# debbiemarkslab/BEAR

Measured on AMD Instinct MI355X. Metric: k-mer contexts/sec (DM-marginal+grad h), k=13, higher is better.
Workload: dtype f64

## Files before the change

### bear_amd/csrc/bear_hip.hip

```cpp
#include "bear_host.h"
#include "kernels_finalize.h"
#include "kernels_rows.h"
#include "kernels_sorted.h"
#include "kernels_plan.h"
#include "kernels_synth.h"
#include "kernels_refmix.h"
#include "kernels_mixplan.h"
#include "kernels_sample.h"
#include "kernels_shuffle.h"
#include "kernels_refplan.h"

#ifdef PLN_STAMPS
#define PLN_DBG_ARG , ws->dbg
#else
#define PLN_DBG_ARG
#endif

extern "C" {

int bear_abi_version(void) { return BEAR_ABI_VERSION; }

const char *bear_strerror(int status) {
  switch (status) {
    case BEAR_OK: return "ok";
// ... 361 lines not shown

static int plan_count_live_rows(bear_plan *p, const plan_scan &sc) {
  unsigned long long h_hist[SRT_NKEY];
  HIP_TRY(hipMemcpy(h_hist, p->hist, sizeof(h_hist), hipMemcpyDeviceToHost));
  unsigned long long live_rows = sc.heavy[1];
  for (int k = 0; k < SRT_NKEY; ++k) live_rows += h_hist[k];
  p->n_live_rows = live_rows;
  return BEAR_OK;
}

static int plan_build(const bear_ws *ws, bear_plan *p) {
  plan_scan sc;
  plan_cut cut;
  int st = plan_scan_table(ws, p, sc);
  if (st != BEAR_OK) return st;
  const char *cut_env = getenv("BEAR_PLAN_CUT");
  st = cut_env && cut_env[0] == 'h' ? cut_on_host(p, sc, cut) : cut_on_device(p, sc, cut);
  if (st != BEAR_OK) return st;
  p->tiles = cut.tiles.release();
  p->n_tiles = cut.n_tiles;
  const uint64_t stream_bytes = cut.off16 * 16 + 1024;
  const uint64_t live_bytes = p->ncol == 5 ? sizeof(uint16_t) * PLN_LIVE_STRIDE * (p->n_tiles + 1) : 0;
  st = plan_fill(ws, p, sc, stream_bytes);
  if (st == BEAR_OK && live_bytes) st = plan_live_lists(ws, p, live_bytes);
  if (st != BEAR_OK) return st;
  HIP_TRY(hipDeviceSynchronize());
  unsigned long long h_used[3] = {0, 0, 0};
  HIP_TRY(hipMemcpy(h_used, sc.cnt.get() + 3, sizeof(h_used), hipMemcpyDeviceToHost));
  for (int k = 0; k < 3; ++k) p->n_heavy[k] = h_used[k];
  st = plan_order_lists(p);
  p->n_live_rows = p->n_rows;
  if (st == BEAR_OK && p->ncol == 5) st = plan_count_live_rows(p, sc);
  p->bytes = stream_bytes + live_bytes + sizeof(pln_tile) * p->n_tiles + sizeof(pln_heavy_col) * sc.heavy[0] +
             sizeof(pln_heavy_row) * sc.heavy[1] + sizeof(uint64_t) * sc.heavy[2];
  return st;
}

int bear_plan_create(bear_ws *ws, const uint32_t *counts, uint64_t n_rows, int ncol, bear_plan **out) {
  if (!out) return BEAR_ERR_INVALID_ARG;
  *out = nullptr;
  int st = check_ws(ws);
  if (st != BEAR_OK) return st;
  if ((ncol != 4 && ncol != 5) || (n_rows && !counts) || misaligned(counts)) return BEAR_ERR_INVALID_ARG;
  plan_guard p(new (std::nothrow) bear_plan());
  if (!p) return BEAR_ERR_NOMEM;
  memset(p.get(), 0, sizeof(bear_plan));
  p->device = ws->device;
  p->ncol = ncol;
  p->n_rows = n_rows;
  p->counts = counts;
  HIP_TRY(hipMalloc(&p->hist, sizeof(unsigned long long) * PLAN_HIST_WORDS));
  HIP_TRY(hipMemset(p->hist, 0, sizeof(unsigned long long) * PLAN_HIST_WORDS));
  if (n_rows) st = plan_build(ws, p.get());
  if (st == BEAR_OK) *out = p.release();
  return st;
}

int bear_plan_destroy(bear_plan *plan) {
  if (!plan) return BEAR_OK;
  int prev = 0;
  (void)hipGetDevice(&prev);
  (void)hipSetDevice(plan->device);
  plan_free(plan);
  (void)hipSetDevice(prev);
  return BEAR_OK;
}

uint64_t bear_plan_bytes(const bear_plan *plan) { return plan ? plan->bytes : 0; }

int bear_plan_create_auto(bear_ws *ws, const uint32_t *counts, uint64_t n_rows, int *rowwise, bear_plan **out) {
  if (rowwise) *rowwise = 0;
  int st = bear_plan_create(ws, counts, n_rows, 5, out);
  if (st != BEAR_OK) return st;
  bear_plan *p = *out;
  const double cells = p->count_total[1], listed = (double)p->n_heavy[0];
  if (!(cells > 0.0) || listed * 2.0 <= cells) return BEAR_OK;
  plan_drop_sorted(p);
  plan_drop_live(p);
  p->ncol = PLAN_ROWS;
  if (rowwise) *rowwise = 1;
  return BEAR_OK;
}
static int launch_prior_rows(bear_ws *ws, const bear_plan *plan, const double *prior, const bear_params &prm, const double *theta,
                             int train_ar, double *out, double *grad_prior, hipStream_t s) {
  const int grid = grid_dense(ws, plan->n_rows);
  const double2 *lt = reinterpret_cast<const double2 *>(ws->logtab);
  const bear_step_io io = ws_io(ws, theta, BEAR_THETA_NET, out);
#define ROWS_LAUNCH(AR, GRAD) \
  hipLaunchKernelGGL((dm_prior_rows_kernel<AR, GRAD>), dim3(grid), dim3(BEAR_THREADS), 0, s, plan->counts, prior, plan->n_rows, prm, grad_prior, lt, \
                     ws->partials, io)
  BEAR_DISPATCH_2(train_ar, grad_prior, ROWS_LAUNCH);
#undef ROWS_LAUNCH
  HIP_TRY(hipGetLastError());
  return BEAR_OK;
}

uint64_t bear_plan_tile_count(const bear_plan *plan) { return plan ? plan->n_tiles : 0; }

int bear_plan_tile_info(const bear_plan *plan, uint64_t first, uint64_t count, uint64_t *row0, uint32_t *rows, uint32_t *items,
                        uint64_t *stream_offset) {
  if (!plan || first + count > plan->n_tiles || (count && (!row0 || !rows || !items || !stream_offset))) return BEAR_ERR_INVALID_ARG;
  if (!count) return BEAR_OK;
  std::vector<pln_tile> h(count);
  int prev = 0;
  (void)hipGetDevice(&prev);
  (void)hipSetDevice(plan->device);
  const hipError_t e = hipMemcpy(h.data(), plan->tiles + first, sizeof(pln_tile) * count, hipMemcpyDeviceToHost);
  (void)hipSetDevice(prev);
  HIP_TRY(e);
  for (uint64_t k = 0; k < count; ++k) {
    row0[k] = h[k].row0;
    rows[k] = h[k].rows_items >> 16;
    items[k] = h[k].rows_items & 0xffffu;
    stream_offset[k] = (uint64_t)h[k].off16 * 16;
  }
  return BEAR_OK;
}

int bear_plan_create_ref(bear_ws *ws, const uint32_t *train, const uint32_t *ref, uint64_t n_rows, bear_plan **out) {
  if (!out) return BEAR_ERR_INVALID_ARG;
  *out = nullptr;
  if ((n_rows && !ref) || misaligned(ref)) return BEAR_ERR_INVALID_ARG;
  bear_plan *created = nullptr;
  int st = bear_plan_create(ws, train, n_rows, 4, &created);
  if (st != BEAR_OK) return st;
  plan_guard p(created);
  p->ref = ref;
  if (p->count_total[1] > 0.0 && (double)p->n_heavy[0] * 2.0 > p->count_total[1]) {
    plan_drop_sorted(p.get());
    p->rows_ref = 1;
    *out = p.release();
    return BEAR_OK;
  }
  HIP_TRY(hipMalloc(&p->hist0_base, sizeof(unsigned long long) * 72));
  unsigned long long *d_meta = p->hist0_base;
  HIP_TRY(hipMemset(d_meta, 0, sizeof(unsigned long long) * 72));
  HIP_TRY(hipMalloc(&p->sum0, sizeof(double)));
  HIP_TRY(hipMemset(p->sum0, 0, sizeof(double)));
  unsigned long long h_meta[72];
  memset(h_meta, 0, sizeof(h_meta));
  const int grid = grid_capped((n_rows + 1023) / 1024, (uint64_t)ws->num_cu * 8);
  if (n_rows) {
    hipLaunchKernelGGL(rpl_build_kernel, dim3(grid), dim3(256), 0, 0, train, ref, n_rows, 0, d_meta, d_meta + 32, d_meta + 64, p->sum0,
                       static_cast<rpl_item *>(nullptr), static_cast<uint32_t *>(nullptr));
    HIP_TRY(hipGetLastError());
    HIP_TRY(hipMemcpy(h_meta, d_meta, sizeof(h_meta), hipMemcpyDeviceToHost));
  }
  unsigned long long run = 0, cur[RPL_NKEY];
  for (int k = 0; k < RPL_NKEY; ++k) {
    cur[k] = run;
    run += h_meta[k];
  }
  p->n_ref_items = run;
  p->n_heavy0 = h_meta[64];
  if (run) HIP_TRY(hipMalloc(&p->ref_items, sizeof(rpl_item) * run));
  if (p->n_heavy0) HIP_TRY(hipMalloc(&p->heavy0, sizeof(uint32_t) * p->n_heavy0));
  HIP_TRY(hipMemcpy(d_meta, cur, sizeof(cur), hipMemcpyHostToDevice));
  HIP_TRY(hipMemset(d_meta + 64, 0, sizeof(unsigned long long)));
  if (n_rows && (run || p->n_heavy0)) {
    hipLaunchKernelGGL(rpl_build_kernel, dim3(grid), dim3(256), 0, 0, train, ref, n_rows, 1, d_meta, d_meta + 32, d_meta + 64, p->sum0,
                       p->ref_items, p->heavy0);
    HIP_TRY(hipGetLastError());
  }
  HIP_TRY(hipDeviceSynchronize());
#ifdef BEAR_DET_BUILD
  for (int k = 0; k < RPL_NKEY && st == BEAR_OK; ++k) st = bear_canonical_order(p->ref_items + cur[k], h_meta[k], 16, 0);
  if (st == BEAR_OK) st = bear_canonical_order(p->heavy0, p->n_heavy0, 4, 0);
  if (st != BEAR_OK) return st;
#endif
  p->hist0 = d_meta + 32;
  p->bytes += sizeof(rpl_item) * p->n_ref_items + sizeof(uint32_t) * p->n_heavy0 + sizeof(unsigned long long) * 72;
  *out = p.release();
  return BEAR_OK;
}

static int launch_prior_plan(bear_ws *ws, const bear_plan *plan, const double *prior, uint64_t n_rows, const bear_params &prm,
                             const double *theta, int train_ar, int prior_normalized, double *out, hipStream_t s) {
  const int grid = grid_plan(ws, plan->n_tiles);
  const double2 *lt = reinterpret_cast<const double2 *>(ws->logtab);
  const bear_step_io io = ws_io(ws, theta, BEAR_THETA_NET, out);
  if (train_ar)
    hipLaunchKernelGGL((dm_prior_plan_kernel<true, true>), dim3(grid), dim3(PLN_THREADS), sizeof(pln_lds_n), s, prior, n_rows, prm,
                       plan_view(plan), lt, ws->partials, io PLN_DBG_ARG);
  else if (prior_normalized)
    hipLaunchKernelGGL((dm_prior_plan_kernel<true, false>), dim3(grid), dim3(PLN_THREADS), sizeof(pln_lds_n), s, prior, n_rows, prm,
                       plan_view(plan), lt, ws->partials, io PLN_DBG_ARG);
  else
    hipLaunchKernelGGL((dm_prior_plan_kernel<false, false>), dim3(grid), dim3(PLN_THREADS), sizeof(pln_lds_n), s, prior, n_rows, prm,
                       plan_view(plan), lt, ws->partials, io PLN_DBG_ARG);
  HIP_TRY(hipGetLastError());
  return BEAR_OK;
}

int bear_dm_prior_plan_f64(bear_ws *ws, const bear_plan *plan, const uint32_t *counts, const double *prior,
                           uint64_t n_rows, double h_signed, double eps, int train_ar, int prior_normalized,
                           double *out, void *stream) {
  int st = check_ws(ws);
  if (st != BEAR_OK) return st;
  if (!plan || !out || (n_rows && (!counts || !prior))) return BEAR_ERR_INVALID_ARG;
  if (check_plan_step(ws, plan, counts, n_rows, 5, true) != BEAR_OK || misaligned(prior) || misaligned8(out)) return BEAR_ERR_INVALID_ARG;
  const bear_params prm = params_net(h_signed, eps);
  if (plan_is_rows(plan)) return launch_prior_rows(ws, plan, prior, prm, nullptr, train_ar, out, nullptr, static_cast<hipStream_t>(stream));
  return launch_prior_plan(ws, plan, prior, n_rows, prm, nullptr, train_ar, prior_normalized, out, static_cast<hipStream_t>(stream));
}

int launch_prior_plan_grad(bear_ws *ws, const bear_plan *plan, const double *prior, const bear_params &prm,
                                  const double *theta, int train_ar, int prior_normalized, double *out, double *grad_prior,
                                  hipStream_t s) {
  const int grid = grid_plan(ws, plan->n_tiles);
  const double2 *lt = reinterpret_cast<const double2 *>(ws->logtab);
  const pln_view pv = plan_view(plan);
  const bear_step_io io = ws_io(ws, theta, BEAR_THETA_NET, out);
  if (train_ar)
    hipLaunchKernelGGL((dm_prior_plan_grad_kernel<true, true>), dim3(grid), dim3(PLN_THREADS), sizeof(pln_lds_g), s, prior, prm, pv, lt,
                       grad_prior, ws->partials, io);
  else if (prior_normalized)
    hipLaunchKernelGGL(dm_prior_plan_grad_inplace_kernel, dim3(grid), dim3(PLN_THREADS), sizeof(pln_lds_gi), s, prior, prm, pv, lt,
                       grad_prior, ws->partials, io);
  else
    hipLaunchKernelGGL((dm_prior_plan_grad_kernel<false, false>), dim3(grid), dim3(PLN_THREADS), sizeof(pln_lds_g), s, prior, prm, pv, lt,
                       grad_prior, ws->partials, io);
  HIP_TRY(hipGetLastError());
  auto fixup_grid = [&](uint64_t nh) { return grid_capped((nh + 255) / 256, (uint64_t)ws->num_cu * 8); };
#define FIXUP(NORM, AR, ROWS, N) \
  hipLaunchKernelGGL((dm_prior_grad_fixup_kernel<NORM, AR, ROWS>), dim3(fixup_grid(N)), dim3(256), 0, s, prior, prm, pv, lt, grad_prior, io)
  if (pv.n_heavy_row && !train_ar) {
    if (prior_normalized) FIXUP(true, false, true, pv.n_heavy_row);
    else FIXUP(false, false, true, pv.n_heavy_row);
  }
  if (pv.n_heavy_col) {
    if (train_ar) FIXUP(true, true, false, pv.n_heavy_col);
    else if (prior_normalized) FIXUP(true, false, false, pv.n_heavy_col);
    else FIXUP(false, false, false, pv.n_heavy_col);
  }
#undef FIXUP
  HIP_TRY(hipGetLastError());
  return BEAR_OK;
}

int bear_dm_prior_plan_grad_f64(bear_ws *ws, const bear_plan *plan, const uint32_t *counts, const double *prior,
                                uint64_t n_rows, double h_signed, double eps, int train_ar, int prior_normalized,
                                double *out, double *grad_prior, void *stream) {
  int st = check_ws(ws);
  if (st != BEAR_OK) return st;
  if (!plan || !out || !grad_prior || (n_rows && (!counts || !prior))) return BEAR_ERR_INVALID_ARG;
  if (check_plan_step(ws, plan, counts, n_rows, 5, true) != BEAR_OK) return BEAR_ERR_INVALID_ARG;
  if (misaligned(prior) || misaligned(grad_prior) || misaligned8(out)) return BEAR_ERR_INVALID_ARG;
  const bear_params prm = params_net(h_signed, eps);
  if (plan_is_rows(plan)) return launch_prior_rows(ws, plan, prior, prm, nullptr, train_ar, out, grad_prior, static_cast<hipStream_t>(stream));
  return launch_prior_plan_grad(ws, plan, prior, prm, nullptr, train_ar, prior_normalized, out, grad_prior,
                                static_cast<hipStream_t>(stream));
}

int bear_dm_prior_plan_dev_f64(bear_ws *ws, const bear_plan *plan, const uint32_t *counts, const double *prior, uint64_t n_rows,
                               const double *h_signed_dev, double eps, int train_ar, int prior_normalized, double *out,
                               double *grad_prior, void *stream) {
  int st = check_ws(ws);
  if (st != BEAR_OK) return st;
  if (!plan || !out || !h_signed_dev || (n_rows && (!counts || !prior))) return BEAR_ERR_INVALID_ARG;
  if (check_plan_step(ws, plan, counts, n_rows, 5, true) != BEAR_OK) return BEAR_ERR_INVALID_ARG;
  if (misaligned(prior) || misaligned(grad_prior) || misaligned8(out)) return BEAR_ERR_INVALID_ARG;
  hipStream_t s = static_cast<hipStream_t>(stream);
  const bear_params only_eps = params_eps(eps);
  if (plan_is_rows(plan)) return launch_prior_rows(ws, plan, prior, only_eps, h_signed_dev, train_ar, out, grad_prior, s);
  if (grad_prior) return launch_prior_plan_grad(ws, plan, prior, only_eps, h_signed_dev, train_ar, prior_normalized, out, grad_prior, s);
  return launch_prior_plan(ws, plan, prior, n_rows, only_eps, h_signed_dev, train_ar, prior_normalized, out, s);
}

int bear_dm_refmix_plan_grad_f64(bear_ws *ws, const bear_plan *plan, const uint32_t *counts, const double *net_rows,
                                 const double *ref_rows, uint64_t n_rows, const double *h_signed_dev, const double *tau_signed_dev,
                                 const double *net_weight_signed_dev, double eps, int train_ar, double *out, double *grad_net_rows,
                                 void *stream) {
  int st = check_ws(ws);
  if (st != BEAR_OK) return st;
  if (!plan || !out || !h_signed_dev || !tau_signed_dev || !net_weight_signed_dev) return BEAR_ERR_INVALID_ARG;
  if (n_rows && (!counts || !net_rows || !ref_rows || !grad_net_rows)) return BEAR_ERR_INVALID_ARG;
  if (check_plan_step(ws, plan, counts, n_rows, 5) != BEAR_OK) return BEAR_ERR_INVALID_ARG;
  if (misaligned(net_rows) || misaligned(ref_rows) || misaligned(grad_net_rows) || misaligned8(out) || misaligned8(h_signed_dev) ||
      misaligned8(tau_signed_dev) || misaligned8(net_weight_signed_dev) || !(eps >= 0.0))
    return BEAR_ERR_INVALID_ARG;
  hipStream_t s = static_cast<hipStream_t>(stream);
  const int grid = grid_plan(ws, plan->n_tiles);
  const double2 *lt = reinterpret_cast<const double2 *>(ws->logtab);
  const pln_view pv = plan_view(plan);
  const bear_step_io io = ws_io(ws, nullptr, BEAR_THETA_REF, out);
#define MIX_LAUNCH(AR)                                                                                                            \
  hipLaunchKernelGGL(dm_refmix_plan_grad_kernel<AR>, dim3(grid), dim3(PLN_THREADS), sizeof(pln_lds_g), s, net_rows, ref_rows, \
                     h_signed_dev, tau_signed_dev, net_weight_signed_dev, eps, pv, lt, grad_net_rows, ws->partials, io)
  BEAR_DISPATCH_1(train_ar, MIX_LAUNCH);
#undef MIX_LAUNCH
  HIP_TRY(hipGetLastError());
  if (pv.n_heavy_col + pv.n_heavy_row) {
    const uint64_t nh = pv.n_heavy_col + pv.n_heavy_row;
    const int g2 = grid_capped((nh + 255) / 256, (uint64_t)ws->num_cu * 4);
#define MIX_FIXUP(AR)                                                                                                      \
  hipLaunchKernelGGL(dm_refmix_fixup_kernel<AR>, dim3(g2), dim3(256), 0, s, net_rows, ref_rows, h_signed_dev, tau_signed_dev, \
                     net_weight_signed_dev, eps, pv, lt, grad_net_rows)
    BEAR_DISPATCH_1(train_ar, MIX_FIXUP);
#undef MIX_FIXUP
    HIP_TRY(hipGetLastError());
  }
  return BEAR_OK;
}


static int launch_ref_plan(bear_ws *ws, const bear_plan *plan, const uint32_t *ref, uint64_t n_rows, const bear_params &prm,
                           const double *theta, int train_ar, double *out, hipStream_t s, const bear_apply_io &apply = NO_APPLY) {
  const double2 *lt = reinterpret_cast<const double2 *>(ws->logtab);
  const bear_step_io io = ws_io(ws, theta, BEAR_THETA_REF, out);
  int grid;
  if (plan->rows_ref) {
    if (plan->ref != ref) return BEAR_ERR_INVALID_ARG;
    grid = grid_dense(ws, n_rows);
#define REF_ROWS(AR) \
  hipLaunchKernelGGL(dm_ref_rows_kernel<AR>, dim3(grid), dim3(BEAR_THREADS), 0, s, plan->counts, ref, n_rows, prm, lt, ws->partials, io, apply)
    BEAR_DISPATCH_1(train_ar, REF_ROWS);
#undef REF_ROWS
  } else if (plan->ref) {
    if (plan->ref != ref) return BEAR_ERR_INVALID_ARG;
    rpl_view rv;
    rv.items = plan->ref_items;
    rv.n_items = plan->n_ref_items;
    rv.hist0 = plan->hist0;
    rv.heavy0 = plan->heavy0;
    rv.n_heavy0 = plan->n_heavy0;
    rv.sum0 = plan->sum0;
    const uint64_t units = (plan->n_ref_items + 63) / 64, want = (units + 3) / 4 + 2, cap = (uint64_t)ws->num_cu * (units > 131072 ? 6 : 4);
    grid = grid_capped(want, cap);
#define REF_ITEMS(AR) \
  hipLaunchKernelGGL(dm_ref_items_kernel<AR>, dim3(grid), dim3(256), 0, s, prm, rv, plan_view(plan), lt, ws->partials, io, apply)
    BEAR_DISPATCH_1(train_ar, REF_ITEMS);
#undef REF_ITEMS
  } else {
    grid = grid_plan(ws, plan->n_tiles);
#define REF_PLAN(AR)                                                                                                                     \
  hipLaunchKernelGGL(dm_ref_plan_kernel<AR>, dim3(grid), dim3(PLN_THREADS), sizeof(pln_lds_r), s, ref, n_rows, prm, plan_view(plan), lt, \
                     ws->partials, io, apply)
    BEAR_DISPATCH_1(train_ar, REF_PLAN);
#undef REF_PLAN
  }
  HIP_TRY(hipGetLastError());
  return BEAR_OK;
}

int bear_dm_ref_plan_f64(bear_ws *ws, const bear_plan *plan, const uint32_t *train, const uint32_t *ref,
                         uint64_t n_rows, double h_signed, double tau_signed, double nu_signed, double eps,
                         int train_ar, double *out, void *stream) {
  int st = check_ws(ws);
  if (st != BEAR_OK) return st;
  if (!plan || !out || (n_rows && (!train || !ref))) return BEAR_ERR_INVALID_ARG;
  if (check_plan_step(ws, plan, train, n_rows, 4) != BEAR_OK || misaligned(ref) || misaligned8(out)) return BEAR_ERR_INVALID_ARG;
  return launch_ref_plan(ws, plan, ref, n_rows, params_ref(h_signed, tau_signed, nu_signed, eps), nullptr, train_ar, out,
                         static_cast<hipStream_t>(stream));
}

static int ref_reduce(bear_ws *ws, const bear_plan *plan, const uint32_t *train, const uint32_t *ref, uint64_t n_rows, const double *theta,
                      double eps, int train_ar, double *packed, hipStream_t s, const bear_apply_io &apply) {
  int st = check_ws(ws);
  if (st != BEAR_OK) return st;
  if (!plan || !packed || !theta || !n_rows || !train || !ref) return BEAR_ERR_INVALID_ARG;
  if (check_plan_step(ws, plan, train, n_rows, 4) != BEAR_OK || misaligned(ref) || misaligned8(packed)) return BEAR_ERR_INVALID_ARG;
  return launch_ref_plan(ws, plan, ref, n_rows, params_eps(eps), theta, train_ar, packed, s, apply);
}

int bear_ref_train_reduce_f64(bear_ws *ws, const bear_plan *plan, const uint32_t *train, const uint32_t *ref, uint64_t n_rows,
                              const double *theta, double eps, int train_ar, double *packed, void *stream) {
  return ref_reduce(ws, plan, train, ref, n_rows, theta, eps, train_ar, packed, static_cast<hipStream_t>(stream), NO_APPLY);
}

int bear_ref_train_step_f64(bear_ws *ws, const bear_plan *plan, const uint32_t *train, const uint32_t *ref, uint64_t n_rows,
                            double *theta, double *adam_m, double *adam_v, double *adam_t, double eps, int train_ar,
                            double learning_rate, double scale, double *out, double *loss_buf, uint64_t loss_cap, void *stream) {
  if (!adam_m || !adam_v || !adam_t) return BEAR_ERR_INVALID_ARG;
  hipStream_t s = static_cast<hipStream_t>(stream);
  if (two_launch_step()) {
    int st = ref_reduce(ws, plan, train, ref, n_rows, theta, eps, train_ar, out, s, NO_APPLY);
    if (st != BEAR_OK) return st;
    return launch_train_apply(theta, 3, out, adam_m, adam_v, adam_t, learning_rate, scale, train_ar, loss_buf, loss_cap, s);
  }
  return ref_reduce(ws, plan, train, ref, n_rows, theta, eps, train_ar, out, s,
                    make_apply(theta, 3, adam_m, adam_v, adam_t, learning_rate, scale, train_ar, loss_buf, loss_cap));
}

int bear_dm_items_f64(bear_ws *ws, const double *x, const uint32_t *c, uint64_t n, int path, double *D, double *P,
                      void *stream) {
  int st = check_ws(ws);
  if (st != BEAR_OK) return st;
  if (n == 0) return BEAR_OK;
  if (!x || !c || !D || !P || path < 0 || path > 2) return BEAR_ERR_INVALID_ARG;
  uint64_t blocks = (n + 255) / 256;
  if (blocks > 0x7fffffffull) return BEAR_ERR_INVALID_ARG;
  hipLaunchKernelGGL(dm_items_kernel, dim3((unsigned)blocks), dim3(256), 0, static_cast<hipStream_t>(stream), x, c, n, path,
                     reinterpret_cast<const double2 *>(ws->logtab), D, P);
  HIP_TRY(hipGetLastError());
  return BEAR_OK;
}

int bear_plan_count_total(const bear_plan *plan, double *total, double *bound) {
  if (!plan) return BEAR_ERR_INVALID_ARG;
  for (int k = 0; k < 3; ++k) {
    if (total) total[k] = plan->count_total[k];
    if (bound) bound[k] = plan->count_bound[k];
  }
  return BEAR_OK;
}

int bear_plan_set_count_bound(bear_plan *plan, const double *bound) {
  if (!plan || !bound) return BEAR_ERR_INVALID_ARG;
  for (int k = 0; k < 3; ++k)
    if (!(bound[k] >= plan->count_total[k]) || !(bound[k] < 0x1p50)) return BEAR_ERR_INVALID_ARG;
  for (int k = 0; k < 3; ++k) plan->count_bound[k] = bound[k];
  return BEAR_OK;
}

static int refmix_grid(const bear_ws *ws, uint64_t n_rows) { return grid_capped((n_rows + RMX_THREADS - 1) / RMX_THREADS, ws_blocks(ws, 2)); }

int bear_ref_mix_forward_f64(bear_ws *ws, const double *net_rows, const double *ref_rows, uint64_t n_rows, const double *tau_signed,
                             const double *net_weight_signed, double *prior, void *stream) {
  int st = check_ws(ws);
  if (st != BEAR_OK) return st;
  if (!tau_signed || !net_weight_signed || misaligned8(tau_signed) || misaligned8(net_weight_signed)) return BEAR_ERR_INVALID_ARG;
  if (n_rows == 0) return BEAR_OK;
  if (!net_rows || !ref_rows || !prior || misaligned(net_rows) || misaligned(ref_rows) || misaligned(prior)) return BEAR_ERR_INVALID_ARG;
  hipLaunchKernelGGL(ref_mix_forward_kernel, dim3(refmix_grid(ws, n_rows)), dim3(RMX_THREADS), 0, static_cast<hipStream_t>(stream),
                     net_rows, ref_rows, tau_signed, net_weight_signed, n_rows, prior);
  HIP_TRY(hipGetLastError());
  return BEAR_OK;
}

int bear_ref_mix_backward_f64(bear_ws *ws, const double *net_rows, const double *ref_rows, const double *grad_prior, uint64_t n_rows,
                              const double *tau_signed, const double *net_weight_signed, double *grad_net_rows, double *grad_scalars,
                              void *stream) {
  int st = check_ws(ws);
  if (st != BEAR_OK) return st;
  if (!tau_signed || !net_weight_signed || !grad_scalars || misaligned8(tau_signed) || misaligned8(net_weight_signed) ||
      misaligned8(grad_scalars))
    return BEAR_ERR_INVALID_ARG;
  hipStream_t s = static_cast<hipStream_t>(stream);
  if (n_rows == 0) {
    HIP_TRY(hipMemsetAsync(grad_scalars, 0, 2 * sizeof(double), s));
    return BEAR_OK;
  }
  if (!net_rows || !ref_rows || !grad_prior || !grad_net_rows || misaligned(net_rows) || misaligned(ref_rows) ||
      misaligned(grad_prior) || misaligned(grad_net_rows))
    return BEAR_ERR_INVALID_ARG;
  hipLaunchKernelGGL(ref_mix_backward_kernel, dim3(refmix_grid(ws, n_rows)), dim3(RMX_THREADS), 0, s, net_rows, ref_rows, grad_prior,
                     tau_signed, net_weight_signed, n_rows, grad_net_rows, ws->partials, ws_arrival(ws), grad_scalars);
  HIP_TRY(hipGetLastError());
  return BEAR_OK;
}

int bear_debug_read_timing(bear_ws *ws, unsigned long long *host, int n_words) {
  if (!ws || !host) return BEAR_ERR_INVALID_ARG;
  HIP_TRY(hipDeviceSynchronize());
  HIP_TRY(hipMemcpy(host, ws->dbg, sizeof(unsigned long long) * (size_t)n_words, hipMemcpyDeviceToHost));
  return BEAR_OK;
}

int bear_debug_occupancy(int which) {
  int nb = -1;
  hipError_t e = which == 0
      ? hipOccupancyMaxActiveBlocksPerMultiprocessor(&nb, dm_prior_sorted_kernel<0>, SRT_THREADS, sizeof(srt_lds_n))
      : hipOccupancyMaxActiveBlocksPerMultiprocessor(&nb, dm_ref_sorted_kernel, SRT_THREADS, sizeof(srt_lds_r));
  return e != hipSuccess ? -1000 - (int)e : nb;
}

int bear_log_gamma_f64(const double *conc, uint64_t n, uint64_t n_samples, uint64_t seed, double *out, void *stream) {
  if (n == 0 || n_samples == 0) return BEAR_OK;
  if (!conc || !out) return BEAR_ERR_INVALID_ARG;
  if (n_samples > (~0ull) / n) return BEAR_ERR_INVALID_ARG;
  const uint64_t total = n * n_samples;
  uint64_t blocks = (total + SMP_THREADS - 1) / SMP_THREADS;
  if (blocks > 65536) blocks = 65536;
  hipLaunchKernelGGL(log_gamma_kernel, dim3((unsigned)blocks), dim3(SMP_THREADS), 0, static_cast<hipStream_t>(stream), conc, n,
                     n_samples, seed, out);
  HIP_TRY(hipGetLastError());
  return BEAR_OK;
}

static int logdir_sample_launch(const uint32_t *counts, const double *prior, uint64_t n_rows, int width, const double *h,
                                int n_h, int with_ar, const double *van, int n_van, int mc_samples, int map, uint64_t seed,
// ... 103 lines not shown
```

### bear_amd/csrc/bear_host.h

```cpp
#pragma once
#include <hip/hip_runtime.h>
#include <math.h>
#include <stdint.h>
#include <stdlib.h>
#include <string.h>

#include <initializer_list>
#include <memory>
#include <new>
#include <vector>

#include "bear_common.h"
#include "bear_dev.h"
#include "bear_levels.h"
#include "plan_common.h"

#define BEAR_INTERNAL __attribute__((visibility("hidden")))

static inline int check_ws(const bear_ws *ws) {
  if (!ws) return BEAR_ERR_INVALID_ARG;
  int dev = -1;
  if (hipGetDevice(&dev) != hipSuccess) return BEAR_ERR_NO_DEVICE;
  if (dev != ws->device) return BEAR_ERR_WRONG_DEVICE;
  return BEAR_OK;
// ... 5 lines not shown

#define BEAR_DISPATCH_2(a, b, F) \
  do {                           \
    if (a) {                     \
      if (b) F(true, true);      \
      else F(true, false);       \
    } else {                     \
      if (b) F(false, true);     \
      else F(false, false);      \
    }                            \
  } while (0)

#define BEAR_DISPATCH_1(a, F) \
  do {                        \
    if (a) F(true);           \
    else F(false);            \
  } while (0)

#define BEAR_DISPATCH_W(width, launch) \
  do {                                 \
    if ((width) == 21) {               \
      constexpr int W = 21;            \
      launch;                          \
    } else {                           \
      constexpr int W = 5;             \
      launch;                          \
    }                                  \
  } while (0)

static inline bear_params params_eps(double eps) {
  bear_params prm;
  memset(&prm, 0, sizeof(prm));
  prm.eps = eps;
  return prm;
}
static inline bear_params params_net(double h_signed, double eps) {
  bear_params prm = params_eps(eps);
  prm.inv_h = 1.0 / exp(h_signed);
  return prm;
}
static inline bear_params params_ref(double h_signed, double tau_signed, double nu_signed, double eps) {
  bear_params prm = params_net(h_signed, eps);
  const double tau = exp(tau_signed), nw = exp(nu_signed);
  prm.E = exp(-tau);
  prm.tauE = tau * prm.E;
  prm.tau = tau;
  prm.V = 1.0 / (nw + 1.0);
  prm.nw = nw;
  return prm;
}

static inline int grid_capped(uint64_t work, uint64_t cap) {
  const uint64_t g = work < cap ? work : cap;
  return g < 1 ? 1 : (int)g;
}
static inline uint64_t ws_blocks(const bear_ws *ws, int per_cu) {
  const uint64_t g = (uint64_t)ws->num_cu * per_cu;
  return g > (uint64_t)ws->max_blocks ? (uint64_t)ws->max_blocks : g;
}
static inline int wide_grid(const bear_ws *ws, uint64_t n_rows, uint64_t tile, int per_cu) {
  return grid_capped((n_rows + tile - 1) / tile, ws_blocks(ws, per_cu));
}

static inline int grid_plan(const bear_ws *ws, uint64_t n_tiles) { return grid_capped(n_tiles, ws_blocks(ws, PLN_BLOCKS_PER_CU)); }

#define BEAR_KFN(...) reinterpret_cast<const void *>(__VA_ARGS__)
static inline int allow_dynamic_lds(std::initializer_list<const void *> kernels, size_t bytes) {
  for (const void *fn : kernels) HIP_TRY(hipFuncSetAttribute(fn, hipFuncAttributeMaxDynamicSharedMemorySize, (int)bytes));
  return BEAR_OK;
}

static inline bear_arrival ws_arrival(bear_ws *ws) {
  if (++ws->epoch == 0u) ws->epoch = 1u;
  return bear_arrival{ws->arrive, ws->epoch};
}

static inline bear_step_io ws_io(bear_ws *ws, const double *theta, int kind, double *out) {
  const bear_arrival a = ws_arrival(ws);
  bear_step_io io;
  io.theta = theta;
  io.kind = kind;
  io.epoch = a.epoch;
  io.out = out;
  io.arrive_word = a.word;
  return io;
}

static inline bool bear_deterministic() {
#ifdef BEAR_DET_BUILD
  return true;
#else
  const char *e = getenv("BEAR_AMD_DETERMINISTIC");
  return e && e[0] && e[0] != '0';
#endif
}

static const bear_apply_io NO_APPLY = {};

static inline bear_apply_io make_apply(double *theta, int n_theta, double *adam_m, double *adam_v, double *adam_t, double learning_rate,
                                       double scale, int train_ar, double *loss_buf, uint64_t loss_cap) {
  bear_apply_io A;
  A.theta = theta;
  A.m = adam_m;
  A.v = adam_v;
  A.t_state = adam_t;
  A.loss_buf = loss_buf;
  A.loss_cap = (unsigned long long)loss_cap;
  A.lr = learning_rate;
  A.scale = scale;
  A.n_theta = n_theta;
  A.train_ar = train_ar;
  return A;
}

static inline bool two_launch_step() {
  const char *e = getenv("BEAR_AMD_TWO_LAUNCH_STEP");
  return e && e[0] && e[0] != '0';
}

struct rpl_item;
struct bear_plan {
  int device;
  int ncol;
  uint64_t n_rows;
  const uint32_t *counts;
  pln_tile *tiles;
  unsigned char *stream;
  pln_heavy_col *heavy_col;
  pln_heavy_row *heavy_row;
  uint64_t *heavy_stop;
  unsigned long long *hist;
  uint16_t *live;
  uint64_t n_tiles;
  uint64_t n_heavy[3];
  int rows_ref;
  uint64_t n_live_rows;
  double count_total[3];
  double count_bound[3];
  uint64_t bytes;
  bear_level_dev cnn_levels[CNN_MAX_LAG];
  int n_cnn_levels, cnn_lag, cnn_fw;
  bear_window_dev cnn_win[CNN_MAX_LAG + 1][CNN_MAX_WIN];
  int n_cnn_win[CNN_MAX_LAG + 1];
  int n_cnn_windows;
  const uint64_t *cnn_codes;
  uint16_t *live2;
  pln_tile *tiles_p, *tiles_u;
  uint64_t n_tiles_p, n_tiles_u;
  const uint64_t *pair_codes;
  int pair_lag;
  const uint32_t *ref;
  rpl_item *ref_items;
  uint64_t n_ref_items, n_heavy0;
  unsigned long long *hist0;
  unsigned long long *hist0_base;
  uint32_t *heavy0;
  double *sum0;
};

static inline pln_view plan_view(const bear_plan *p) {
  pln_view v;
  v.tiles = p->tiles;
  v.stream = p->stream;
  v.heavy_col = p->heavy_col;
  v.heavy_row = p->heavy_row;
  v.heavy_stop = p->heavy_stop;
  v.hist = p->hist;
  v.hist_big = p->hist + 2 * SRT_NKEY;
  v.big_in_hist = 1;
  v.live = p->live;
  v.live2 = p->live2;
  v.subset = 0;
  v.n_tiles = p->n_tiles;
  v.n_heavy_col = p->n_heavy[0];
  v.n_heavy_row = p->n_heavy[1];
  v.n_heavy_stop = p->n_heavy[2];
  return v;
}

#define PLAN_ROWS 15
static inline bool plan_is_rows(const bear_plan *p) { return p->ncol == PLAN_ROWS; }
static inline int check_plan_step(const bear_ws *ws, const bear_plan *plan, const uint32_t *counts, uint64_t n_rows, int ncol,
                                  bool or_rows = false) {
  if (plan->ncol != ncol && !(or_rows && plan_is_rows(plan))) return BEAR_ERR_INVALID_ARG;
  if (plan->counts != counts || plan->n_rows != n_rows || plan->device != ws->device) return BEAR_ERR_INVALID_ARG;
  return BEAR_OK;
}

BEAR_INTERNAL int linear_ws_setup(bear_ws *ws);
BEAR_INTERNAL int cnn_ws_setup(bear_ws *ws);
BEAR_INTERNAL int eval_ws_setup(bear_ws *ws);
BEAR_INTERNAL void plan_unpair(bear_plan *plan);
BEAR_INTERNAL void plan_drop_cnn_levels(bear_plan *plan);

extern "C" {
BEAR_INTERNAL int launch_prior_plan_grad(bear_ws *ws, const bear_plan *plan, const double *prior, const bear_params &prm,
                                         const double *theta, int train_ar, int prior_normalized, double *out, double *grad_prior,
                                         hipStream_t s);
BEAR_INTERNAL int launch_train_apply(double *theta, int n_theta, const double *packed, double *adam_m, double *adam_v, double *adam_t,
                                     double learning_rate, double scale, int train_ar, double *loss_buf, uint64_t loss_cap, hipStream_t s);
}
```

### bear_amd/csrc/kernels_refplan.h

```cpp
#pragma once
#include "kernels_plan.h"

#define RPL_NKEY 32
#define RPL_HEAVY_KEY 24

struct rpl_item {
  uint32_t c, rb;
  double R;
};
static_assert(sizeof(rpl_item) == 16, "one 16-byte lane load per record");

struct rpl_view {
  const rpl_item *items;
  uint64_t n_items;
  const unsigned long long *hist0;
  const uint32_t *heavy0;
  uint64_t n_heavy0;
  const double *sum0;
};

__global__ __launch_bounds__(256) void rpl_build_kernel(const uint32_t *__restrict__ train, const uint32_t *__restrict__ ref, uint64_t n_rows,
                                                        int fill, unsigned long long *__restrict__ bucket,
                                                        unsigned long long *__restrict__ hist0, unsigned long long *__restrict__ n_heavy0,
                                                        double *__restrict__ sum0, rpl_item *__restrict__ items,
                                                        uint32_t *__restrict__ heavy0) {
  constexpr int RPT = 4;
  __shared__ uint32_t s_bucket[RPL_NKEY], s_hist0[RPL_NKEY];
  __shared__ unsigned long long s_at[RPL_NKEY];
  __shared__ double s_sum;
  const uint32_t tid = threadIdx.x;
  const uint64_t per_block = (n_rows + gridDim.x - 1) / gridDim.x;
  const uint64_t r_begin = (uint64_t)blockIdx.x * per_block, r_end = r_begin + per_block < n_rows ? r_begin + per_block : n_rows;
  for (uint64_t base = r_begin; base < r_end; base += 256u * RPT) {
    if (tid < RPL_NKEY) s_bucket[tid] = s_hist0[tid] = 0u;
    if (tid == 0) s_sum = 0.0;
    __syncthreads();
    uint32_t c[RPT][4], rb[RPT][4], rank[RPT][4];
    double R[RPT];
    double my_sum = 0.0;
#pragma unroll
    for (int k = 0; k < RPT; ++k) {
      const uint64_t row = base + tid + 256u * k;
      R[k] = -1.0;
#pragma unroll
      for (int b = 0; b < 4; ++b) c[k][b] = rb[k][b] = rank[k][b] = 0u;
      if (row < r_end) {
        uint64_t rs = 0;
#pragma unroll
        for (int b = 0; b < 4; ++b) {
          c[k][b] = train[row * 5 + b];
          rb[k][b] = ref[row * 5 + b];
          rs += rb[k][b];
        }
        R[k] = (double)rs;
#pragma unroll
        for (int b = 0; b < 4; ++b) {
          if (c[k][b] == 0u) continue;
          if (rs == 0) {
            my_sum += (double)c[k][b];
            if (c[k][b] <= SRT_CL) {
              if (!fill) atomicAdd(&s_hist0[c[k][b] - 1], 1u);
            } else if (fill) {
              heavy0[atomicAdd(n_heavy0, 1ull)] = c[k][b];
            } else {
              atomicAdd(n_heavy0, 1ull);
            }
          } else {
            const uint32_t key = (c[k][b] > SRT_CL ? SRT_CL + 1u : c[k][b]) - 1u;
            rank[k][b] = atomicAdd(&s_bucket[key], 1u);
          }
        }
      }
    }
    if (!fill && my_sum != 0.0) atomicAdd(&s_sum, my_sum);
    __syncthreads();
    if (tid < RPL_NKEY && !fill) {
      if (s_bucket[tid]) atomicAdd(&bucket[tid], (unsigned long long)s_bucket[tid]);
      if (s_hist0[tid]) atomicAdd(&hist0[tid], (unsigned long long)s_hist0[tid]);
    }
    if (!fill && tid == 0 && s_sum != 0.0) atomicAdd(sum0, s_sum);
    if (fill) {
      if (tid < RPL_NKEY) s_at[tid] = s_bucket[tid] ? atomicAdd(&bucket[tid], (unsigned long long)s_bucket[tid]) : 0ull;
      __syncthreads();
#pragma unroll
      for (int k = 0; k < RPT; ++k) {
        if (!(R[k] > 0.0)) continue;
#pragma unroll
        for (int b = 0; b < 4; ++b) {
          if (c[k][b] == 0u) continue;
          const uint32_t key = (c[k][b] > SRT_CL ? SRT_CL + 1u : c[k][b]) - 1u;
          rpl_item it;
          it.c = c[k][b];
          it.rb = rb[k][b];
          it.R = R[k];
          items[s_at[key] + rank[k][b]] = it;
        }
      }
    }
    __syncthreads();
  }
}

template <bool AR>
__global__ __launch_bounds__(256) void dm_ref_items_kernel(bear_params prm_arg, rpl_view rv, pln_view pv, const double2 *__restrict__ logtab_g,
                                                           double *__restrict__ partials, const bear_step_io io, const bear_apply_io apply) {
  __shared__ double2 s_log[BEAR_LOGTAB_N];
  const bear_params prm = bear_params_of(prm_arg, io);
  const uint32_t tid = threadIdx.x, lane = tid & 63u;
  const double u = prm.inv_h, eps = prm.eps;
  const double A = u + 5.0 * eps;
  const double x4 = prm.nw * prm.V * u + eps;
  const double VU = prm.V * u;
  const double tau = prm.tau;
  const double w2c = tau * (eps + 0.25 * VU);
  const double nwV = prm.nw * prm.V;
  double acc[4] = {0.0, 0.0, 0.0, 0.0};
  if (tid < BEAR_LOGTAB_N) s_log[tid] = logtab_g[tid];
  __syncthreads();
  auto alpha_from = [&](double rb, double R) {
    const double dev = __builtin_fma(rb + eps, bear_rcp(R), -0.25);
    return __builtin_fma(__builtin_fma(prm.E, dev, 0.25), VU, eps);
  };
  auto accumulate = [&](double x, double m, const bear_dp &o) {
    const double w1 = eps - x, P = m * o.P;
    acc[0] = __builtin_fma(m, o.D, acc[0]);
    acc[1] = __builtin_fma(w1, P, acc[1]);
    acc[2] = __builtin_fma(__builtin_fma(-tau, x, w2c), P, acc[2]);
    acc[3] = __builtin_fma(nwV * w1, P, acc[3]);
  };
  auto accumulate_ar = [&](double rb, double R, double c) {
    const double dev = __builtin_fma(rb + eps, bear_rcp(R), -0.25);
    const double f = __builtin_fma(prm.E, dev, 0.25) * prm.V;
    const double p = f + eps;
    const double dLdf = c * bear_rcp(p);
    acc[0] = __builtin_fma(c, bear_log_tab(p, s_log), acc[0]);
    acc[2] = __builtin_fma(dLdf, -prm.tauE * dev * prm.V, acc[2]);
    acc[3] = __builtin_fma(dLdf, -nwV * f, acc[3]);
  };
  const uint64_t n_units = (rv.n_items + 63u) >> 6;
  const uint64_t wave_g = ((uint64_t)blockIdx.x * 256u + tid) >> 6, n_waves = ((uint64_t)gridDim.x * 256u) >> 6;
  for (uint64_t un = wave_g; un < n_units; un += n_waves) {
    const uint64_t i = un * 64u + lane;
    rpl_item it;
    it.c = 0u;
    it.rb = 0u;
    it.R = 1.0;
    if (i < rv.n_items) it = rv.items[i];
    const double R = it.R + 4.0 * eps;
    if (AR) {
      if (it.c) accumulate_ar((double)it.rb, R, (double)it.c);
      continue;
    }
    const bool heavy = it.c > SRT_CL;
    const uint32_t cc = heavy ? SRT_CL + 1u : it.c;
    const uint32_t occ = (un + 1u) * 64u <= rv.n_items ? 64u : (uint32_t)(rv.n_items - un * 64u);
    const uint32_t cmin = occ == 64u ? (uint32_t)__builtin_amdgcn_readlane((int)cc, 0) : 0u;
    const uint32_t cmax = (uint32_t)__builtin_amdgcn_readlane((int)cc, (int)(occ - 1u));
    const double x[1] = {alpha_from((double)it.rb, R)};
    const uint32_t ci[1] = {heavy ? 0u : it.c};
    bear_dp o[1];
    srt_light<1>(x, ci, cmin > SRT_CL ? SRT_CL : cmin, cmax > SRT_CL ? SRT_CL : cmax, s_log, o);
    if (__builtin_amdgcn_ballot_w64(heavy)) {
      if (heavy) o[0] = srt_general_fast(x[0], (double)it.c, s_log);
    }
    if (it.c) accumulate(x[0], 1.0, o[0]);
  }
  const uint64_t gtid = (uint64_t)blockIdx.x * 256u + tid, gsz = (uint64_t)gridDim.x * 256u;
  const double R0 = 4.0 * eps;
  if (AR) {
    if (gtid == 0) accumulate_ar(0.0, R0, rv.sum0[0]);
    const double f4 = nwV, p4 = f4 + eps;
    double c4sum = 0.0;
    if (blockIdx.x == 0 && tid < SRT_CL) c4sum = (double)(tid + 1) * (double)pv.hist[SRT_NKEY + tid];
    for (uint64_t i = gtid; i < pv.n_heavy_stop; i += gsz) c4sum += (double)pv.heavy_stop[i];
    acc[0] = __builtin_fma(c4sum, bear_log_tab(p4, s_log), acc[0]);
    acc[3] = __builtin_fma(c4sum * bear_rcp(p4), nwV * (1.0 - f4), acc[3]);
    __syncthreads();
    block_finish<4>(acc, partials, io, apply);
    return;
  }
  const double x0 = alpha_from(0.0, R0);
  if (blockIdx.x == 0 && tid < SRT_CL) {
    const double m = (double)rv.hist0[tid];
    if (m != 0.0) accumulate(x0, m, srt_general_fast(x0, (double)(tid + 1), s_log));
  }
  for (uint64_t i = gtid; i < rv.n_heavy0; i += gsz) accumulate(x0, 1.0, srt_general_fast(x0, (double)rv.heavy0[i], s_log));
  for (uint64_t i = gtid; i < pv.n_heavy_row; i += gsz) {
    const double n = pv.heavy_row[i].n;
    if (pln_in_big_hist(pv, n)) continue;
    const bear_dp o = srt_general_fast(A, n, s_log);
    acc[0] -= o.D;
    acc[1] = __builtin_fma(u, o.P, acc[1]);
  }
  pln_big_totals(pv, A, u, gtid, gsz, s_log, acc[0], acc[1]);
  for (uint64_t i = gtid; i < pv.n_heavy_stop; i += gsz) {
    const bear_dp o = srt_general_fast(x4, (double)pv.heavy_stop[i], s_log);
    acc[0] += o.D;
    acc[1] = __builtin_fma(eps - x4, o.P, acc[1]);
    acc[3] = __builtin_fma(VU * nwV, o.P, acc[3]);
  }
  if (blockIdx.x == 1 % gridDim.x && tid < SRT_CL) {
    const double mn = (double)pv.hist[tid], m4 = (double)pv.hist[SRT_NKEY + tid];
    const bear_dp on = srt_general_fast(A, (double)(tid + 1), s_log), o4 = srt_general_fast(x4, (double)(tid + 1), s_log);
    acc[0] -= mn * on.D;
    acc[1] = __builtin_fma(u * mn, on.P, acc[1]);
    const double P4 = m4 * o4.P;
    acc[0] += m4 * o4.D;
    acc[1] = __builtin_fma(eps - x4, P4, acc[1]);
    acc[3] = __builtin_fma(VU * nwV, P4, acc[3]);
  }
  __syncthreads();
  block_finish<4>(acc, partials, io, apply);
}
```

Baseline: 139.0 billion.

## Memoize per-chunk (rb,R) pair results in LDS and stream ref items via ring

The ref-items kernel now splits items into light and heavy (Stirling) ranges. Light items are processed in per-block chunks where the results for small (rb,R) pairs at the chunk's one or two count values are precomputed into an LDS table, so most records only need a lookup. Records are staged through a per-wave LDS ring using async DMA. Heavy items are handled in a separate pass, which alternates ordering across blocks to balance CU load, and occupancy is pinned through launch bounds. This adds chunk-sizing logic on the host, more LDS use, and extra block syncs.

```diff
diff --git a/bear_amd/csrc/bear_hip.hip b/bear_amd/csrc/bear_hip.hip
--- a/bear_amd/csrc/bear_hip.hip
+++ b/bear_amd/csrc/bear_hip.hip
@@ -537,6 +537,7 @@
     run += h_meta[k];
   }
   p->n_ref_items = run;
+  p->n_ref_light = cur[RPL_HEAVY_KEY];
   p->n_heavy0 = h_meta[64];
   if (run) HIP_TRY(hipMalloc(&p->ref_items, sizeof(rpl_item) * run));
   if (p->n_heavy0) HIP_TRY(hipMalloc(&p->heavy0, sizeof(uint32_t) * p->n_heavy0));
@@ -710,8 +711,10 @@
     rv.heavy0 = plan->heavy0;
     rv.n_heavy0 = plan->n_heavy0;
     rv.sum0 = plan->sum0;
-    const uint64_t units = (plan->n_ref_items + 63) / 64, want = (units + 3) / 4 + 2, cap = (uint64_t)ws->num_cu * (units > 131072 ? 6 : 4);
+    const uint64_t units = (plan->n_ref_items + 63) / 64, want = (units + 3) / 4 + 2, cap = (uint64_t)ws->num_cu * (units > 131072 ? RPL_OCC : 4);
     grid = grid_capped(want, cap);
+    rv.n_light = plan->n_ref_light;
+    rpl_chunking(train_ar ? units : (plan->n_ref_light + 63) / 64, (uint32_t)grid, &rv.upw, &rv.n_chunks);
 #define REF_ITEMS(AR) \
   hipLaunchKernelGGL(dm_ref_items_kernel<AR>, dim3(grid), dim3(256), 0, s, prm, rv, plan_view(plan), lt, ws->partials, io, apply)
     BEAR_DISPATCH_1(train_ar, REF_ITEMS);
diff --git a/bear_amd/csrc/bear_host.h b/bear_amd/csrc/bear_host.h
--- a/bear_amd/csrc/bear_host.h
+++ b/bear_amd/csrc/bear_host.h
@@ -181,6 +181,7 @@
   const uint32_t *ref;
   rpl_item *ref_items;
   uint64_t n_ref_items, n_heavy0;
+  uint64_t n_ref_light;
   unsigned long long *hist0;
   unsigned long long *hist0_base;
   uint32_t *heavy0;
diff --git a/bear_amd/csrc/kernels_refplan.h b/bear_amd/csrc/kernels_refplan.h
--- a/bear_amd/csrc/kernels_refplan.h
+++ b/bear_amd/csrc/kernels_refplan.h
@@ -10,14 +10,57 @@
 };
 static_assert(sizeof(rpl_item) == 16, "one 16-byte lane load per record");
 
+#ifndef RPL_RTAB
+#define RPL_RTAB 14
+#endif
+#define RPL_NPAIR (RPL_RTAB * (RPL_RTAB + 3) / 2)
+#ifndef RPL_RING
+#define RPL_RING 1
+#endif
+#ifndef RPL_UPW
+#define RPL_UPW 12
+#endif
+#ifndef RPL_OCC
+#define RPL_OCC 6
+#endif
+#ifndef RPL_STIRLING_SPLIT
+#define RPL_STIRLING_SPLIT 1
+#endif
+#define RPL_MIN_CHUNKS 2
+#define RPL_MAX_CHUNKS 16
+static_assert(2 * RPL_NPAIR <= 256, "a chunk's table is filled in one pass of the block");
+static_assert((RPL_RING & (RPL_RING - 1)) == 0 && RPL_RING <= 8, "ring slots by mask; pln_wait_all_but's ladder");
+
 struct rpl_view {
   const rpl_item *items;
   uint64_t n_items;
+  uint64_t n_light;
+  uint32_t upw, n_chunks;
   const unsigned long long *hist0;
   const uint32_t *heavy0;
   uint64_t n_heavy0;
   const double *sum0;
 };
+
+inline void rpl_chunking(uint64_t n_tab_units, uint32_t grid, uint32_t *upw, uint32_t *n_chunks) {
+  const uint64_t per_wave = (n_tab_units + 4ull * grid - 1) / (4ull * grid);
+  uint64_t m0 = (per_wave + RPL_UPW / 2) / RPL_UPW;
+  m0 = m0 < RPL_MIN_CHUNKS ? RPL_MIN_CHUNKS : m0 > RPL_MAX_CHUNKS ? RPL_MAX_CHUNKS : m0;
+  uint64_t best_u = 1;
+  double best_fill = -1.0;
+  for (uint64_t m = m0; m <= m0 + 2 && m <= RPL_MAX_CHUNKS; ++m) {
+    uint64_t u = (n_tab_units + 4ull * m * grid - 1) / (4ull * m * grid);
+    u = u < 1 ? 1 : u > 0x1000000u ? 0x1000000u : u;
+    const uint64_t chunks = (n_tab_units + 4 * u - 1) / (4 * u), rounds = (chunks + grid - 1) / grid;
+    const double fill = rounds ? (double)chunks / (double)(rounds * grid) : 1.0;
+    if (fill > best_fill + 0.02) {
+      best_fill = fill;
+      best_u = u;
+    }
+  }
+  *upw = (uint32_t)best_u;
+  *n_chunks = (uint32_t)((n_tab_units + 4 * best_u - 1) / (4 * best_u));
+}
 
 __global__ __launch_bounds__(256) void rpl_build_kernel(const uint32_t *__restrict__ train, const uint32_t *__restrict__ ref, uint64_t n_rows,
                                                         int fill, unsigned long long *__restrict__ bucket,
@@ -102,7 +145,7 @@
 }
 
 template <bool AR>
-__global__ __launch_bounds__(256) void dm_ref_items_kernel(bear_params prm_arg, rpl_view rv, pln_view pv, const double2 *__restrict__ logtab_g,
+__global__ __launch_bounds__(256, RPL_OCC) void dm_ref_items_kernel(bear_params prm_arg, rpl_view rv, pln_view pv, const double2 *__restrict__ logtab_g,
                                                            double *__restrict__ partials, const bear_step_io io, const bear_apply_io apply) {
   __shared__ double2 s_log[BEAR_LOGTAB_N];
   const bear_params prm = bear_params_of(prm_arg, io);
@@ -128,42 +171,173 @@
     acc[2] = __builtin_fma(__builtin_fma(-tau, x, w2c), P, acc[2]);
     acc[3] = __builtin_fma(nwV * w1, P, acc[3]);
   };
-  auto accumulate_ar = [&](double rb, double R, double c) {
-    const double dev = __builtin_fma(rb + eps, bear_rcp(R), -0.25);
+  auto ar_pair = [&](double rb, double R, double &dev, double &logp, double &rp) {
+    dev = __builtin_fma(rb + eps, bear_rcp(R), -0.25);
+    const double p = __builtin_fma(prm.E, dev, 0.25) * prm.V + eps;
+    logp = bear_log_tab(p, s_log);
+    rp = bear_rcp(p);
+  };
+  auto ar_terms = [&](double dev, double logp, double rp, double c) {
     const double f = __builtin_fma(prm.E, dev, 0.25) * prm.V;
-    const double p = f + eps;
-    const double dLdf = c * bear_rcp(p);
-    acc[0] = __builtin_fma(c, bear_log_tab(p, s_log), acc[0]);
+    const double dLdf = c * rp;
+    acc[0] = __builtin_fma(c, logp, acc[0]);
     acc[2] = __builtin_fma(dLdf, -prm.tauE * dev * prm.V, acc[2]);
     acc[3] = __builtin_fma(dLdf, -nwV * f, acc[3]);
   };
+  auto accumulate_ar = [&](double rb, double R, double c) {
+    double dev, logp, rp;
+    ar_pair(rb, R, dev, logp, rp);
+    ar_terms(dev, logp, rp, c);
+  };
+  __shared__ double s_tx[2 * RPL_NPAIR];
+  __shared__ double2 s_tdp[2 * RPL_NPAIR];
+  __shared__ __attribute__((aligned(16))) rpl_item s_ring[4][RPL_RING][64];
+  const uint32_t wave = srt_uniform(tid >> 6);
   const uint64_t n_units = (rv.n_items + 63u) >> 6;
-  const uint64_t wave_g = ((uint64_t)blockIdx.x * 256u + tid) >> 6, n_waves = ((uint64_t)gridDim.x * 256u) >> 6;
-  for (uint64_t un = wave_g; un < n_units; un += n_waves) {
-    const uint64_t i = un * 64u + lane;
-    rpl_item it;
-    it.c = 0u;
-    it.rb = 0u;
-    it.R = 1.0;
-    if (i < rv.n_items) it = rv.items[i];
-    const double R = it.R + 4.0 * eps;
-    if (AR) {
-      if (it.c) accumulate_ar((double)it.rb, R, (double)it.c);
-      continue;
-    }
-    const bool heavy = it.c > SRT_CL;
-    const uint32_t cc = heavy ? SRT_CL + 1u : it.c;
-    const uint32_t occ = (un + 1u) * 64u <= rv.n_items ? 64u : (uint32_t)(rv.n_items - un * 64u);
-    const uint32_t cmin = occ == 64u ? (uint32_t)__builtin_amdgcn_readlane((int)cc, 0) : 0u;
-    const uint32_t cmax = (uint32_t)__builtin_amdgcn_readlane((int)cc, (int)(occ - 1u));
-    const double x[1] = {alpha_from((double)it.rb, R)};
-    const uint32_t ci[1] = {heavy ? 0u : it.c};
-    bear_dp o[1];
-    srt_light<1>(x, ci, cmin > SRT_CL ? SRT_CL : cmin, cmax > SRT_CL ? SRT_CL : cmax, s_log, o);
-    if (__builtin_amdgcn_ballot_w64(heavy)) {
-      if (heavy) o[0] = srt_general_fast(x[0], (double)it.c, s_log);
-    }
-    if (it.c) accumulate(x[0], 1.0, o[0]);
+  const uint64_t n_tab_units = AR ? n_units : (rv.n_light + 63u) >> 6;
+  const uint32_t upw = rv.upw, n_chunks = rv.n_chunks;
+  const uint64_t chunk_units = 4ull * upw;
+  uint32_t issued = 0, done = 0, pk = blockIdx.x, pi = 0;
+  auto issue = [&]() {
+    if (pk >= n_chunks) return;
+    const uint64_t un = (uint64_t)pk * chunk_units + 4u * pi + wave;
+    if (un >= n_tab_units) {
+      pk = n_chunks;
+      return;
+    }
+    const uint64_t left = rv.n_items - un * 64u;
+    pln_dma_piece(&s_ring[wave][issued & (RPL_RING - 1)][0], rv.items + un * 64u, left >= 64u ? 1024u : (uint32_t)left * 16u, 0u, lane);
+    ++issued;
+    if (++pi == upw) {
+      pi = 0;
+      pk += gridDim.x;
+    }
+  };
+  auto next_record = [&](uint64_t un) {
+    const uint32_t younger = issued - done - 1u;
+    if (younger >= RPL_RING - 1u) pln_wait_all_but(RPL_RING - 1u);
+    else pln_wait_all_but(younger);
+    rpl_item it = s_ring[wave][done & (RPL_RING - 1)][lane];
+    asm volatile("s_waitcnt lgkmcnt(0)" ::: "memory");
+    ++done;
+    issue();
+    if (un * 64u + lane >= rv.n_items) {
+      it.c = 0u;
+      it.rb = 0u;
+      it.R = 1.0;
+    }
+    return it;
+  };
+  auto pair_of = [&](uint32_t e, uint32_t &rb, uint32_t &Rt) {
+    uint32_t base = 0;
+    Rt = 1;
+    while (e - base > Rt) {
+      base += Rt + 1u;
+      ++Rt;
+    }
+    rb = e - base;
+  };
+  auto pair_index = [&](const rpl_item &it) {
+#ifdef RPL_NO_TABLE
+    return (uint32_t)RPL_NPAIR;
+#endif
+    const bool small = it.R <= (double)RPL_RTAB;
+    const uint32_t Rt = small ? (uint32_t)it.R : 0u;
+    return Rt >= 1u && it.rb <= Rt ? Rt * (Rt + 1u) / 2u - 1u + it.rb : (uint32_t)RPL_NPAIR;
+  };
+  auto stirling_units = [&]() {
+    const uint64_t wave_g = (uint64_t)blockIdx.x * 4u + wave, n_waves = (uint64_t)gridDim.x * 4u;
+    for (uint64_t un = n_tab_units + wave_g; un < n_units; un += n_waves) {
+      const uint64_t i = un * 64u + lane;
+      if (i < rv.n_items) {
+        const rpl_item it = rv.items[i];
+        const double x = alpha_from((double)it.rb, it.R + 4.0 * eps);
+        accumulate(x, 1.0, srt_general_fast(x, (double)it.c, s_log));
+      }
+    }
+  };
+  const uint32_t cu_stride = gridDim.x >= RPL_OCC ? gridDim.x / RPL_OCC : 1u;
+  const bool stirling_first = RPL_STIRLING_SPLIT && ((blockIdx.x / cu_stride) & 1u);
+  if (!AR && stirling_first) stirling_units();
+#pragma unroll 1
+  for (int k = 0; k < RPL_RING; ++k) issue();
+  if (AR) {
+    if (blockIdx.x < n_chunks) {
+      if (tid < RPL_NPAIR) {
+        uint32_t rb, Rt;
+        pair_of(tid, rb, Rt);
+        double dev, logp, rp;
+        ar_pair((double)rb, (double)Rt + 4.0 * eps, dev, logp, rp);
+        s_tx[tid] = dev;
+        s_tdp[tid] = make_double2(logp, rp);
+      }
+      srt_sync();
+    }
+    for (uint32_t k = blockIdx.x; k < n_chunks; k += gridDim.x) {
+#pragma unroll 1
+      for (uint32_t i = 0; i < upw; ++i) {
+        const uint64_t un = (uint64_t)k * chunk_units + 4u * i + wave;
+        if (un >= n_tab_units) break;
+        const rpl_item it = next_record(un);
+        const uint32_t e = pair_index(it);
+        const bool hit = e < RPL_NPAIR;
+        const double2 lr = s_tdp[hit ? e : 0u];
+        if (it.c && hit) ar_terms(s_tx[hit ? e : 0u], lr.x, lr.y, (double)it.c);
+        if (__builtin_amdgcn_ballot_w64(it.c && !hit)) {
+          if (it.c && !hit) accumulate_ar((double)it.rb, it.R + 4.0 * eps, (double)it.c);
+        }
+      }
+    }
+  } else {
+    for (uint32_t k = blockIdx.x; k < n_chunks; k += gridDim.x) {
+      const uint64_t r_first = (uint64_t)k * chunk_units * 64u;
+      const uint64_t r_last = (r_first + chunk_units * 64u < rv.n_light ? r_first + chunk_units * 64u : rv.n_light) - 1u;
+      const __attribute__((address_space(4))) rpl_item *ic = (const __attribute__((address_space(4))) rpl_item *)(uintptr_t)rv.items;
+      const uint32_t c0 = ic[r_first].c, c_end = ic[r_last].c;
+      const uint32_t c1 = c_end != c0 ? c_end : 0u;
+      const uint32_t n_entries = c1 ? 2u * RPL_NPAIR : (uint32_t)RPL_NPAIR;
+      srt_sync();
+      if (wave * 64u < n_entries) {
+        const uint32_t e = tid < RPL_NPAIR ? tid : tid - RPL_NPAIR;
+        uint32_t rb, Rt;
+        pair_of(e < RPL_NPAIR ? e : 0u, rb, Rt);
+        const double xe[1] = {alpha_from((double)rb, (double)Rt + 4.0 * eps)};
+        const uint32_t ce[1] = {tid < n_entries ? (tid < RPL_NPAIR ? c0 : c1) : 0u};
+        bear_dp oe[1];
+        srt_light<1>(xe, ce, 0u, c1 ? c1 : c0, s_log, oe);
+        if (tid < n_entries) {
+          s_tx[tid] = xe[0];
+          s_tdp[tid] = make_double2(oe[0].D, oe[0].P);
+        }
+      }
+      srt_sync();
+#pragma unroll 1
+      for (uint32_t i = 0; i < upw; ++i) {
+        const uint64_t un = (uint64_t)k * chunk_units + 4u * i + wave;
+        if (un >= n_tab_units) break;
+        const rpl_item it = next_record(un);
+        const uint32_t ep = pair_index(it);
+        const bool hit = it.c && ep < RPL_NPAIR && (it.c == c0 || it.c == c1);
+        if (hit) {
+          const uint32_t e = ep + (it.c == c0 ? 0u : (uint32_t)RPL_NPAIR);
+          const double2 dp = s_tdp[e];
+          accumulate(s_tx[e], 1.0, bear_dp{dp.x, dp.y});
+        }
+        const bool own = it.c && !hit;
+        if (__builtin_amdgcn_ballot_w64(own)) {
+          const bool heavy = it.c > SRT_CL;
+          const double xo[1] = {alpha_from((double)it.rb, it.R + 4.0 * eps)};
+          const uint32_t co[1] = {own && !heavy ? it.c : 0u};
+          bear_dp oo[1] = {bear_dp{0.0, 0.0}};
+          if (__builtin_amdgcn_ballot_w64(co[0] != 0u)) srt_light<1>(xo, co, 0u, c1 ? c1 : c0, s_log, oo);
+          if (__builtin_amdgcn_ballot_w64(heavy)) {
+            if (heavy) oo[0] = srt_general_fast(xo[0], (double)it.c, s_log);
+          }
+          if (own) accumulate(xo[0], 1.0, oo[0]);
+        }
+      }
+    }
+    if (!stirling_first) stirling_units();
   }
   const uint64_t gtid = (uint64_t)blockIdx.x * 256u + tid, gsz = (uint64_t)gridDim.x * 256u;
   const double R0 = 4.0 * eps;
```

Result: no change. 139.0 billion (median of 2 runs) (+0.1%).
